# fdarmon/wild_deep_mvs

Hardware: AMD Instinct MI355X
Metric: cost-volume voxels/sec (BxDxHxW), MVSNet hot path (higher is better)
Workload: dtype bf16

## Files before the change

### wild_deep_mvs_amd/csrc/pscv_common.h

```cpp
#pragma once
#include <hip/hip_runtime.h>
#include <stdint.h>
#include <stdio.h>
#include <stdarg.h>

#include "../../include/pscv.h"

namespace pscv {

void set_error(const char* fmt, ...);

hipError_t ensure_dyn_lds(const void* kernel, int bytes);
int device_cu_count();

struct Knob {
    int process;
    int id;
    operator int() const;
    void set(int v) { __atomic_store_n(&process, v, __ATOMIC_RELAXED); }
};
#define PSCV_KNOB_TABLE(X)                      \
    X("warp_q2", g_warp_q2, 1)                  \
    X("warp_lpv", g_warp_lpv_override, 0)       \
    X("warp_ppd", g_warp_ppd_override, 0)       \
    X("warp_tiled", g_warp_tiled, 1)            \
    X("warp_tile", g_warp_tile, 0)              \
    X("warp_gc_lds", g_warp_gc_lds, 1)          \
    X("warp_lds_pad", g_warp_lds_pad, 0)        \
    X("warp_bwd_direct", g_warp_bwd_direct, 0)  \
    X("sweep_dc", g_sweep_dc, 0)                \
    X("sweepc_slots", g_sweepc_slots, 0)        \
    X("sweepc_pd", g_sweepc_pd, 0)              \
    X("sweep_th16", g_sweep_th16, 0)            \
    X("sweep_kdm", g_sweep_kdm, 0)              \
    X("sweep_kdm_pd", g_sweep_kdm_pd, 0)        \
    X("c1_sweep", g_c1_sweep, 1)                \
    X("c1_nb", g_c1_nb, 0)                      \
    X("conv_s2_sweep", g_conv_s2_sweep, 1)      \
    X("s2s_slots", g_s2s_slots, 0)              \
    X("block8_slots", g_block8_slots, 0)        \
    X("conv2d_wlds", g_conv2d_wlds, 1)          \
// ... 264 lines not shown
```

### wild_deep_mvs_amd/csrc/pscv_host.cpp

```cpp
#include <stdarg.h>
#include <stdio.h>
#include <string.h>

#include <functional>
#include <mutex>
#include <unordered_map>

#include "pscv_common.h"

namespace pscv {

namespace {
struct DynLdsKey {
    const void* kernel;
    int dev;
    bool operator==(const DynLdsKey& o) const { return kernel == o.kernel && dev == o.dev; }
};
struct DynLdsHash {
    size_t operator()(const DynLdsKey& k) const { return std::hash<const void*>()(k.kernel) * 31u + std::hash<int>()(k.dev); }
};
struct DynLdsSlot { const void* kernel; int dev; int bytes; };
constexpr int DYN_LDS_SLOTS = 64;
thread_local DynLdsSlot g_dyn_lds_tl[DYN_LDS_SLOTS];
}
// ... 37 lines not shown
}

int device_cu_count() {
    constexpr int MAXDEV = 64;
    static int cached[MAXDEV];
    int dev = 0;
    if (hipGetDevice(&dev) != hipSuccess) return -1;
    if (dev >= 0 && dev < MAXDEV) {
        const int c = __atomic_load_n(&cached[dev], __ATOMIC_RELAXED);
        if (c > 0) return c;
    }
    int n = 0;
    if (hipDeviceGetAttribute(&n, hipDeviceAttributeMultiprocessorCount, dev) != hipSuccess || n <= 0) return -1;
    if (dev >= 0 && dev < MAXDEV) __atomic_store_n(&cached[dev], n, __ATOMIC_RELAXED);
    return n;
}

static thread_local char g_err[512] = "";

void set_error(const char* fmt, ...) {
    va_list ap;
    va_start(ap, fmt);
    vsnprintf(g_err, sizeof(g_err), fmt, ap);
    va_end(ap);
}

#define PSCV_KNOB_ID(key, sym, def) KNOB_##sym,
enum { PSCV_KNOB_TABLE(PSCV_KNOB_ID) KNOB_COUNT };
#undef PSCV_KNOB_ID
#define PSCV_KNOB_DEFINE(key, sym, def) Knob sym = {def, KNOB_##sym};
// ... 211 lines not shown
```

### wild_deep_mvs_amd/csrc/warp_common.h

```cpp
#pragma once
#include "pscv_common.h"

namespace pscv {

struct WarpArgs {
    const void* ref;
    const void* src[PSCV_MAX_SRC];
    const float* cams;
    const float* depth;
    void* out;
    long depth_bstride;
    long out_view_stride;
    int n_src, B, h, w, hs, ws, D;
    int depth_per_pixel;
    int ppd;
    int npb_batch;
    int n_dchunks;
    int variant;
    float temp;
    float sx, sy;
    float xlo, xhi, ylo, yhi;
    int ref_y0;
    int* mode_hist;
};

template <int N> struct VecF { float v[N]; };

template <typename T, int CPL> __device__ __forceinline__ VecF<CPL> load_chan(const T* p) {
    VecF<CPL> r;
#pragma unroll
    for (int k = 0; k < CPL / 8; ++k) {
        const f32x8 t = Elem<T>::load8(p + 8 * k);
#pragma unroll
        for (int j = 0; j < 8; ++j) r.v[8 * k + j] = t.v[j];
    }
    return r;
}
// ... 154 lines not shown
```

### wild_deep_mvs_amd/csrc/warp_cost.hip

```cpp
#include <string.h>

#include "warp_common.h"

namespace pscv {

template <typename TIn, typename TOut, int C, int LPV, int GEOM, int COST>
__global__ __launch_bounds__(256, 4) void warp_cost_kernel(const WarpArgs a) {
    constexpr int CPL = C / LPV;
    constexpr int PPB = 256 / LPV;
    constexpr int PIXB = C * (int)sizeof(TIn);
    constexpr int RQ = (GEOM == PSCV_GEOM_HOMOG) ? 2 : 1;
    static_assert(CPL % 8 == 0, "a lane owns whole 8-channel groups");

    const int wg = xcd_remap(blockIdx.x, gridDim.x);
    const int pb = __builtin_amdgcn_readfirstlane(wg / a.n_dchunks);
    const int dc = __builtin_amdgcn_readfirstlane(wg - pb * a.n_dchunks);

    const int b = __builtin_amdgcn_readfirstlane(pb / a.npb_batch);
    const int pbb = __builtin_amdgcn_readfirstlane(pb - b * a.npb_batch);

    const int tid = threadIdx.x;
    __shared__ float cam_lds[PSCV_MAX_SRC * PSCV_CAM_FLOATS];
    extern __shared__ __attribute__((aligned(16))) float4 ray_lds[];
    for (int i = tid; i < a.n_src * PSCV_CAM_FLOATS; i += 256) {
// ... 248 lines not shown
extern "C" int pscv_warp_cost_rows(const void* ref, const void* const* srcs, int n_src, const float* cams,
                                   const float* depth, long depth_bstride, int depth_per_pixel, int geom, int cost,
                                   float temp, void* out, int B, int C, int h, int w, int hs, int ws, int D, int in_dtype,
                                   int out_dtype, int ref_y0, void* stream) {
    using namespace pscv;
    PSCV_CHECK_ARG(ref_y0 >= 0 && ref_y0 < (1 << 20), "pscv_warp_cost_rows: ref_y0=%d", ref_y0);
    PSCV_CHECK_ARG(n_src >= 1 && n_src <= PSCV_MAX_SRC, "pscv_warp_cost: n_src=%d outside [1,%d]", n_src, PSCV_MAX_SRC);
    PSCV_CHECK_ARG(srcs && cams && depth && out, "pscv_warp_cost: null pointer argument");
    PSCV_CHECK_ARG(cost == PSCV_COST_WARP_ONLY || cost == PSCV_COST_VARIANCE_PARTIAL || ref, "pscv_warp_cost: ref is required for cost mode %d", cost);
    PSCV_CHECK_ARG(cost != PSCV_COST_VARIANCE_PARTIAL || out_dtype == PSCV_F32, "pscv_warp_cost: partial sums are written in fp32");
    PSCV_CHECK_ARG(B > 0 && h > 0 && w > 0 && hs > 1 && ws > 1 && D > 0, "pscv_warp_cost: bad sizes");
    PSCV_CHECK_ARG(C % 8 == 0, "pscv_warp_cost: C=%d must be a multiple of 8", C);
    PSCV_CHECK_ARG((long)hs * ws < (1L << 24) && (long)hs * ws * C * 4 < (1L << 32), "pscv_warp_cost: source map %dx%dx%d too large", hs, ws, C);
    WarpArgs a;
    a.mode_hist = nullptr;
    a.ref_y0 = ref_y0;
    a.ref = ref;
    for (int i = 0; i < PSCV_MAX_SRC; ++i) a.src[i] = i < n_src ? srcs[i] : nullptr;
    for (int i = 0; i < n_src; ++i) PSCV_CHECK_ARG(srcs[i], "pscv_warp_cost: srcs[%d] is null", i);
    a.cams = cams;
    a.depth = depth;
    a.out = out;
    a.depth_bstride = depth_bstride;
    a.n_src = n_src; a.B = B; a.h = h; a.w = w; a.hs = hs; a.ws = ws; a.D = D;
    a.depth_per_pixel = depth_per_pixel;
    a.temp = temp;
    a.variant = 0;
    const long vol = (long)B * D * h * w;
    a.out_view_stride = cost == PSCV_COST_GROUPCORR ? vol * (C / 4) : vol * C;
    if (geom == PSCV_GEOM_PROJ) {
// ... 27 lines not shown
```

### wild_deep_mvs_amd/csrc/warp_cost_tiled.hip

```cpp
#include <type_traits>

#include "warp_common.h"
#include "warp_lds.h"

namespace pscv {

#ifndef WL_TILE_H
#define WL_TILE_H 4
#endif
constexpr int WL_T = 8;
constexpr int WL_TH = WL_TILE_H;
constexpr int WL_THREADS = 64 * WL_TH;
constexpr int WL_PG = WL_TH / 2;
constexpr int WL_ARENA = WL_TH == 8 ? 636 : 316;
constexpr int WL_HI = WL_ARENA * 64;
constexpr int WL_STAGE_ROWS = 8;
constexpr int WL_BOX_H = WL_STAGE_ROWS * (WL_THREADS / 64 / WL_MAX_SRC);
constexpr int WL_NSETS = 7;
constexpr int WL_TABLE = 2 * WL_HI;
constexpr int WL_LDS = WL_TABLE + WL_NSETS * WL_MAX_SRC * 16 + 32;
static_assert(WL_LDS <= (WL_TH == 8 ? 81920 : 40960), "two / four blocks per CU");


__device__ __forceinline__ void wl_blend8(const wl_f4 (&t)[8], const float (&w)[4], float (&o)[8]) {
    o[0] = t[0].x * w[0]; o[1] = t[0].y * w[0]; o[2] = t[0].z * w[0]; o[3] = t[0].w * w[0];
    o[4] = t[1].x * w[0]; o[5] = t[1].y * w[0]; o[6] = t[1].z * w[0]; o[7] = t[1].w * w[0];
#pragma unroll
    for (int k = 1; k < 4; ++k) {
        o[0] = fmaf(t[2 * k].x, w[k], o[0]); o[1] = fmaf(t[2 * k].y, w[k], o[1]);
        o[2] = fmaf(t[2 * k].z, w[k], o[2]); o[3] = fmaf(t[2 * k].w, w[k], o[3]);
        o[4] = fmaf(t[2 * k + 1].x, w[k], o[4]); o[5] = fmaf(t[2 * k + 1].y, w[k], o[5]);
        o[6] = fmaf(t[2 * k + 1].z, w[k], o[6]); o[7] = fmaf(t[2 * k + 1].w, w[k], o[7]);
    }
}

__device__ __forceinline__ wl_f4 wl_tap(const unsigned char* lsm, unsigned off) { return *reinterpret_cast<const wl_f4*>(lsm + off); }

template <typename TOut> __device__ __forceinline__ void wl_store8(char* p, const float (&o)[8]) {
    if constexpr (sizeof(TOut) == 4) {
        *reinterpret_cast<float4*>(p) = make_float4(o[0], o[1], o[2], o[3]);
        *reinterpret_cast<float4*>(p + 16) = make_float4(o[4], o[5], o[6], o[7]);
    } else {
        *reinterpret_cast<uint4*>(p) = make_uint4(wl_pack2<TOut>(o[0], o[1]), wl_pack2<TOut>(o[2], o[3]),
                                                   wl_pack2<TOut>(o[4], o[5]), wl_pack2<TOut>(o[6], o[7]));
    }
}


template <typename TIn, typename TOut, int GEOM, int COST>
__global__ __launch_bounds__(WL_THREADS, 4) void warp_cost_lds_kernel(const WarpArgs a) {
    constexpr int C = 32, PIXB = 64;
    constexpr int OB = (int)sizeof(TOut);
    constexpr bool VAR = COST == PSCV_COST_VARIANCE || COST == PSCV_COST_VARIANCE_CVP;
    static_assert(GEOM == PSCV_GEOM_PROJ, "PROJ geometry (three depth-independent ray terms per (view, pixel))");
    extern __shared__ __attribute__((aligned(16))) unsigned char lsm[];

    const int dc = blockIdx.y;
    int b, tyi, txi;
    if (!wl_tile_decode<WL_T, WL_TH>(a, b, tyi, txi)) return;

    __builtin_amdgcn_s_setprio(3);
    __builtin_amdgcn_s_setreg((1 - 1) << 11 | 23 << 6 | 1, 1);
    const int tid = threadIdx.x;
    const int wave = __builtin_amdgcn_readfirstlane(tid >> 6), lane = tid & 63;
    const int x0t = txi * WL_T, y0t = tyi * WL_TH;
    const int d0 = dc * a.ppd, d1 = min(a.D, d0 + a.ppd);
    const float* const depth_b = a.depth + (long)b * a.depth_bstride;
    const int n_src = a.n_src;
    int* const table = reinterpret_cast<int*>(lsm + WL_TABLE);

    const float dlane = depth_b[min(d0 + lane, d1 - 1)];

    const int quad = lane >> 2, l = lane & 3;
    const int pl = (2 * (wave % WL_PG) + (quad >> 3)) * 8 + ((0x73261540u >> (4 * (quad & 7))) & 7);
// ... 8 lines not shown
    {
        const float* cam = a.cams + ((long)min(l, n_src - 1) * a.B + b) * PSCV_CAM_FLOATS;
        rx = fmaf(cam[1], py, cam[0] * px) + cam[2];
        ry = fmaf(cam[4], py, cam[3] * px) + cam[5];
        rz = fmaf(cam[7], py, cam[6] * px) + cam[8];
        tx = cam[9]; ty_ = cam[10]; tz = cam[11];
    }
    float rf[8], rf2[8];
    {
        const f32x8 t = Elem<TIn>::load8(reinterpret_cast<const TIn*>(a.ref) + ((long)b * hw + pflat) * C + l * 8);
#pragma unroll
        for (int j = 0; j < 8; ++j) { rf[j] = t.v[j]; rf2[j] = t.v[j] * t.v[j]; }
    }

    const int nplanes = d1 - d0;
    auto split_size = [](int m) { return m >= 4 ? ((m / 2 + 1) & ~1) : m; };
    const int hsz = split_size(nplanes);
    const int q0 = split_size(hsz), q2 = split_size(nplanes - hsz);
    if (wave < WL_MAX_SRC) {
        const int k = wave;
        const float inf = __builtin_inff();
        const bool inq0 = lane < q0, inq1 = lane >= q0 && lane < hsz, inq2 = lane >= hsz && lane < hsz + q2, inq3 = lane >= hsz + q2;
        const float qmin0 = wl_wave_reduce<false>(inq0 ? dlane : inf), qmax0 = wl_wave_reduce<true>(inq0 ? dlane : -inf);
        const float qmin1 = wl_wave_reduce<false>(inq1 ? dlane : inf), qmax1 = wl_wave_reduce<true>(inq1 ? dlane : -inf);
        const float qmin2 = wl_wave_reduce<false>(inq2 ? dlane : inf), qmax2 = wl_wave_reduce<true>(inq2 ? dlane : -inf);
        const float qmin3 = wl_wave_reduce<false>(inq3 ? dlane : inf), qmax3 = wl_wave_reduce<true>(inq3 ? dlane : -inf);
        const float dmin1 = fminf(qmin0, qmin1), dmax1 = fmaxf(qmax0, qmax1);
        const float dmin2 = hsz < nplanes ? fminf(qmin2, qmin3) : dmin1, dmax2 = hsz < nplanes ? fmaxf(qmax2, qmax3) : dmax1;
        const float dmin0 = fminf(dmin1, dmin2), dmax0 = fmaxf(dmax1, dmax2);
        const int set = min(lane >> 3, WL_NSETS - 1);
        const int corner = lane & 7;
        const float cx = (corner & 1) ? (float)min(x0t + WL_T - 1, a.w - 1) : (float)x0t;
        const float cy = (float)(((corner & 2) ? min(y0t + WL_TH - 1, a.h - 1) : y0t) + a.ref_y0);
        const float dlo = set == 0 ? dmin0 : set == 1 ? dmin1 : set == 2 ? dmin2 : set == 3 ? qmin0 : set == 4 ? qmin1 : set == 5 ? qmin2 : qmin3;
        const float dhi = set == 0 ? dmax0 : set == 1 ? dmax1 : set == 2 ? dmax2 : set == 3 ? qmax0 : set == 4 ? qmax1 : set == 5 ? qmax2 : qmax3;
        const float d = (corner & 4) ? dhi : dlo;
        int cX0 = 0, cY0 = 0, cX1 = -1, cY1 = -1, pitch = 4, mode = WL_ZERO;
        if (k < n_src) {
            typedef const __attribute__((address_space(4))) float* wl_cf;
            wl_cf cam = (wl_cf)(a.cams + ((long)k * a.B + b) * PSCV_CAM_FLOATS);
            const float ax = fmaf(cam[1], cy, cam[0] * cx) + cam[2];
            const float ay = fmaf(cam[4], cy, cam[3] * cx) + cam[5];
            const float az = fmaf(cam[7], cy, cam[6] * cx) + cam[8];
            const float hx = fmaf(ax, d, cam[9]), hy = fmaf(ay, d, cam[10]), hz = fmaf(az, d, cam[11]);
            const float inv_z = __builtin_amdgcn_rcpf(hz);
            const float u = hx * inv_z, v = hy * inv_z;
            const float okf = (hz > 1e-6f && fabsf(u) < 1e6f && fabsf(v) < 1e6f) ? 1.0f : 0.0f;
            const float umin = wl_reduce8<false>(u), umax = wl_reduce8<true>(u);
            const float vmin = wl_reduce8<false>(v), vmax = wl_reduce8<true>(v);
            const bool ok = wl_reduce8<false>(okf) != 0.0f;
            const float sl = 1.0f / 32.0f;
            const int X0 = (int)floorf(umin - sl), X1 = (int)floorf(umax + sl) + 1;
            const int Y0 = (int)floorf(vmin - sl), Y1 = (int)floorf(vmax + sl) + 1;
            mode = WL_DIRECT;
            if (ok) {
                const bool outside = X1 < 0 || Y1 < 0 || X0 > a.ws - 1 || Y0 > a.hs - 1;
                const bool inside = X0 >= 0 && Y0 >= 0 && X1 <= a.ws - 1 && Y1 <= a.hs - 1;
                cX0 = max(X0, 0); cX1 = min(X1, a.ws - 1); cY0 = max(Y0, 0); cY1 = min(Y1, a.hs - 1);
                const int bw = cX1 - cX0 + 1, bh = cY1 - cY0 + 1;
                pitch = (bw + 3) & ~3;
                if (outside) { mode = WL_ZERO; cX0 = 0; cY0 = 0; cX1 = -1; cY1 = -1; pitch = 4; }
                else if (bw <= 16 && bh <= WL_BOX_H) mode = inside ? WL_FAST : WL_GEN;
                else { cX0 = 0; cY0 = 0; cX1 = -1; cY1 = -1; pitch = 4; }
            } else { cX0 = 0; cY0 = 0; cX1 = -1; cY1 = -1; pitch = 4; }
        }
        if (corner == 0 && lane < 8 * WL_NSETS)
            *reinterpret_cast<uint4*>(table + (set * WL_MAX_SRC + k) * 4) =
                make_uint4(((unsigned)cX0 & 0xffffu) | ((unsigned)cY0 << 16), ((unsigned)cX1 & 0xffffu) | ((unsigned)cY1 << 16),
                           (unsigned)pitch | ((unsigned)mode << 16), 0u);
    }
    __syncthreads();

    int bPitch[WL_MAX_SRC], bMode[WL_MAX_SRC], bBase[WL_MAX_SRC], bX0[WL_MAX_SRC], bY0[WL_MAX_SRC], bX1[WL_MAX_SRC], bY1[WL_MAX_SRC];
    bool any_gen = false;
    auto read_records = [&](int set) -> bool {
        int used = 0;
        bool direct = false;
        any_gen = false;
#pragma unroll
        for (int k = 0; k < WL_MAX_SRC; ++k) {
            const uint4 rec = *reinterpret_cast<const uint4*>(table + (set * WL_MAX_SRC + k) * 4);
            const int rx = __builtin_amdgcn_readfirstlane((int)rec.x), ry = __builtin_amdgcn_readfirstlane((int)rec.y);
            const int rz = __builtin_amdgcn_readfirstlane((int)rec.z);
            bX0[k] = (short)(rx & 0xffff); bY0[k] = rx >> 16;
            bX1[k] = (short)(ry & 0xffff); bY1[k] = ry >> 16;
            bPitch[k] = rz & 0xffff;
            int mode = rz >> 16;
            const int need = bPitch[k] * (bY1[k] - bY0[k] + 1);
            if ((mode == WL_FAST || mode == WL_GEN) && used + need > WL_ARENA) mode = WL_DIRECT;
            bBase[k] = used;
            if (mode == WL_FAST || mode == WL_GEN) used += need;
            bMode[k] = mode;
            any_gen = any_gen || mode == WL_GEN;
            direct = direct || (k < n_src && mode == WL_DIRECT);
        }
        return direct;
    };
    unsigned long plan = 0;
    int nseg = 0;
    auto push = [&](int set, int pa, int pb) { plan |= (unsigned long)((unsigned)set | (unsigned)pa << 3 | (unsigned)pb << 9) << (16 * nseg); ++nseg; };
    if (!read_records(0) || !(hsz < nplanes) || a.variant == 1) {
        push(0, 0, nplanes);
    } else {
        const bool quarters = a.variant != 3;
        if (read_records(1) && q0 < hsz && quarters) { push(3, 0, q0); push(4, q0, hsz); } else push(1, 0, hsz);
        if (read_records(2) && q2 < nplanes - hsz && quarters) { push(5, hsz, hsz + q2); push(6, hsz + q2, nplanes); } else push(2, hsz, nplanes);
    }
    for (int sub = 0; sub < nseg; ++sub) {
    const unsigned seg = (unsigned)(plan >> (16 * sub)) & 0xffffu;
    if (sub) {
        __syncthreads();
        __builtin_amdgcn_s_setprio(3);
    }
    read_records((int)(seg & 7u));
    const int s0 = d0 + (int)((seg >> 3) & 63u), s1 = d0 + (int)(seg >> 9);
    if (a.mode_hist && tid == 0) {
#pragma unroll
        for (int k = 0; k < WL_MAX_SRC; ++k)
            if (k < n_src) atomicAdd(a.mode_hist + k * 4 + bMode[k], 1);
    }
    const int sel = l;
    int mX0 = bX0[0], mY0 = bY0[0], mX1 = bX1[0], mY1 = bY1[0], mpitch = bPitch[0], mbase = bBase[0];
#pragma unroll
    for (int k = 1; k < WL_MAX_SRC; ++k)
        if (sel == k) { mX0 = bX0[k]; mY0 = bY0[k]; mX1 = bX1[k]; mY1 = bY1[k]; mpitch = bPitch[k]; mbase = bBase[k]; }
    const int meb = mbase - mY0 * mpitch - mX0;

    {
        constexpr int WPV = WL_THREADS / 64 / WL_MAX_SRC;
// ... 190 lines not shown
            for (int j = 0; j < 8; ++j) { const float m = __fmul_rn(invN, s[j]); o[j] = fmaf(invN, q[j], -__fmul_rn(m, m)); }
        } else {
            const float inv = 1.0f / (sum_e + 1e-6f);
#pragma unroll
            for (int j = 0; j < 8; ++j) o[j] = s[j] * inv;
        }
#pragma unroll
        for (int j = 0; j < 8; ++j) asm volatile("" : "+v"(o[j]));
        if (active) wl_store8<TOut>(out + ((unsigned long)b * a.D + d) * plane_bytes + lane_out, o);
    }
    }
}

template <typename TIn, typename TOut, int COST>
static int wl_launch(const WarpArgs& a, dim3 grid, hipStream_t st) {
    const int lds = min(WL_LDS + 1024 * max(0, (int)g_warp_lds_pad), 160 * 1024);
    return launch("pscv_warp_cost(lds)", warp_cost_lds_kernel<TIn, TOut, PSCV_GEOM_PROJ, COST>, grid, dim3(WL_THREADS), lds, st, a);
}

template <typename TIn, typename TOut>
static int wl_dispatch(const WarpArgs& a, int cost, dim3 grid, hipStream_t st) {
    if (cost == PSCV_COST_VARIANCE) return wl_launch<TIn, TOut, PSCV_COST_VARIANCE>(a, grid, st);
    if (cost == PSCV_COST_VARIANCE_CVP) return wl_launch<TIn, TOut, PSCV_COST_VARIANCE_CVP>(a, grid, st);
    if (cost == PSCV_COST_SOFTMIN) return wl_launch<TIn, TOut, PSCV_COST_SOFTMIN>(a, grid, st);
    return 1;
}

int* g_wl_mode_hist = nullptr;

int warp_cost_tiled_try(WarpArgs& a, int C, int geom, int cost, int in_dtype, int out_dtype, int ppd_override, hipStream_t st) {
    if (a.depth_per_pixel || geom != PSCV_GEOM_PROJ) return 1;
    if (out_dtype != in_dtype && out_dtype != PSCV_F32) return 1;
    if (a.n_src < 1 || a.n_src > WL_MAX_SRC) return 1;
    dim3 grid;
    const int rc = wl_plan("pscv_warp_cost(lds)", a, C, in_dtype, WL_T, WL_TH, ppd_override, a.D >= 96 ? 48 : 32, 64, grid);
    if (rc) return rc;
    a.variant = g_warp_tile;
    a.mode_hist = g_wl_mode_hist;
    return with_warp_types<false>("pscv_warp_cost(lds)", in_dtype, out_dtype, [&](auto ti, auto to) {
        return wl_dispatch<typename decltype(ti)::type, typename decltype(to)::type>(a, cost, grid, st);
    });
}

}

extern "C" void pscv_debug_wl_mode_hist(int* hist) { pscv::g_wl_mode_hist = hist; }
extern "C" int pscv_debug_wl_occupancy(int* blocks_per_cu, int* lds_bytes, int* threads) {
    auto kern = pscv::warp_cost_lds_kernel<pscv::f16_t, pscv::f16_t, PSCV_GEOM_PROJ, PSCV_COST_VARIANCE>;
    (void)pscv::ensure_dyn_lds(reinterpret_cast<const void*>(kern), pscv::WL_LDS);
    *lds_bytes = pscv::WL_LDS;
    *threads = pscv::WL_THREADS;
    return (int)hipOccupancyMaxActiveBlocksPerMultiprocessor(blocks_per_cu, kern, pscv::WL_THREADS, pscv::WL_LDS);
}
```

### wild_deep_mvs_amd/csrc/warp_lds.h

```cpp
#pragma once
#include "warp_common.h"

namespace pscv {

constexpr int WL_MAX_SRC = 4;
typedef float wl_f4 __attribute__((ext_vector_type(4)));

template <int CTRL> __device__ __forceinline__ int wl_dpp_i(int x) { return __builtin_amdgcn_mov_dpp(x, CTRL, 0xf, 0xf, true); }
template <int CTRL> __device__ __forceinline__ float wl_dpp_f(float x) {
    return __builtin_bit_cast(float, wl_dpp_i<CTRL>(__builtin_bit_cast(int, x)));
}


template <bool MAX> __device__ __forceinline__ float wl_mm(float a, float b) { return MAX ? fmaxf(a, b) : fminf(a, b); }
template <bool MAX, int CTRL, int ROWMASK = 0xf> __device__ __forceinline__ float wl_red_step(float x) {
    const int xi = __builtin_bit_cast(int, x);
    const float y = __builtin_bit_cast(float, __builtin_amdgcn_update_dpp(xi, xi, CTRL, ROWMASK, 0xf, false));
    return wl_mm<MAX>(x, y);
}
template <bool MAX> __device__ __forceinline__ float wl_reduce8(float x) {
    x = wl_red_step<MAX, 0xB1>(x);
    x = wl_red_step<MAX, 0x4E>(x);
    return wl_red_step<MAX, 0x141>(x);
}
// ... 9 lines not shown
    if constexpr (Half16<TOut>::dtype == PSCV_F16) {
        h2_t v;
        v[0] = (_Float16)lo;
        v[1] = (_Float16)hi;
        return __builtin_bit_cast(uint32_t, v);
    } else {
        return Half16<TOut>::pack(lo, hi);
    }
}
constexpr int WL_DIRECT = 0;
constexpr int WL_GEN = 1;
constexpr int WL_FAST = 2;
constexpr int WL_ZERO = 3;


template <int T, int TH> __device__ __forceinline__ bool wl_tile_decode(const WarpArgs& a, int& b, int& tyi, int& txi) {
    const int tpx = gridDim.x >> 3;
    const int ntx = (a.w + T - 1) / T, nty = (a.h + TH - 1) / TH;
    const int tile = ((int)blockIdx.x & 7) * tpx + ((int)blockIdx.x >> 3);
    if (tile >= a.B * nty * ntx) return false;
    const int trow = (int)(((float)tile + 0.5f) * (1.0f / (float)ntx));
    txi = tile - trow * ntx;
    b = (int)(((float)trow + 0.5f) * (1.0f / (float)nty));
    tyi = trow - b * nty;
    return true;
}

inline int wl_plan(const char* what, WarpArgs& a, int C, int in_dtype, int T, int TH, int ppd_override, int ppd_default, int ppd_max, dim3& grid) {
    if (C != 32 || (in_dtype != PSCV_F16 && in_dtype != PSCV_BF16)) return 1;
    if (a.ws > 16384 || a.hs > 16384) return 1;
    const long tiles = (long)a.B * ((a.h + TH - 1) / TH) * ((a.w + T - 1) / T);
    if (tiles >= (1L << 22)) return 1;
    int ppd = ppd_override > 0 ? min((ppd_override + 1) & ~1, ppd_max) : ppd_default;
    while (ppd > 4 && tiles * ((a.D + ppd - 1) / ppd) < 1024) ppd >>= 1;
    a.ppd = ppd;
    a.n_dchunks = (a.D + ppd - 1) / ppd;
    const long nblk = tiles * a.n_dchunks;
    if (nblk <= 0 || nblk > 0x7fffffffL) { set_error("%s: bad grid %ld", what, nblk); return -1; }
    grid = dim3(8 * (unsigned)((tiles + 7) / 8), a.n_dchunks);
    return 0;
// ... 4 lines not shown
```

### wild_deep_mvs_amd/graph.py

```python
from __future__ import annotations

from typing import Any, Dict, Tuple

import torch
import torch.nn as nn


def _sig(x) -> Any:
    if isinstance(x, torch.Tensor):
        return ("T", tuple(x.shape), str(x.dtype), str(x.device))
    if isinstance(x, (list, tuple)):
        return (type(x).__name__,) + tuple(_sig(v) for v in x)
    if isinstance(x, dict):
        return ("D",) + tuple((k, _sig(v)) for k, v in sorted(x.items()))
    return ("V", repr(x))


def _clone_static(x):
    if isinstance(x, torch.Tensor):
        return x.detach().clone()
    if isinstance(x, (list, tuple)):
        return type(x)(_clone_static(v) for v in x)
    if isinstance(x, dict):
        return {k: _clone_static(v) for k, v in x.items()}
# ... 49 lines not shown
        wkey = _weights_key(self.model)
        entry = self._graphs.get(key)
        if entry is not None and entry[3] != wkey:
            entry = None
        if entry is None:
            static_args, static_kwargs = _clone_static(args), _clone_static(kwargs)
            with torch.no_grad():
                side = torch.cuda.Stream()
                side.wait_stream(torch.cuda.current_stream())
                with torch.cuda.stream(side):
                    for _ in range(self.warmup):
                        self.model(*static_args, **static_kwargs)
                torch.cuda.current_stream().wait_stream(side)
                torch.cuda.synchronize()
                graph = torch.cuda.CUDAGraph()
                with torch.cuda.graph(graph, capture_error_mode="thread_local"):
                    static_out = self.model(*static_args, **static_kwargs)
            entry = (graph, (static_args, static_kwargs), static_out, wkey)
            self._graphs[key] = entry
        graph, (static_args, static_kwargs), static_out, _ = entry
        _copy_in(static_args, args)
        _copy_in(static_kwargs, kwargs)
        graph.replay()
        return _clone_out(static_out)


import functools
import operator
import sys
import threading
from collections import OrderedDict
# ... 112 lines not shown
                    state["seen"][key] = True
                    while len(state["seen"]) > 64:
                        state["seen"].popitem(last=False)
                    eager = True
            if not eager and entry is None:
                static_args, static_kwargs = _clone_static(args), _clone_static(kwargs)
                try:
                    with torch.no_grad():
                        side = torch.cuda.Stream()
                        side.wait_stream(torch.cuda.current_stream())
                        with torch.cuda.stream(side):
                            forward(self, *static_args, **static_kwargs)
                        torch.cuda.current_stream().wait_stream(side)
                        torch.cuda.synchronize()
                        graph = torch.cuda.CUDAGraph()
                        with torch.cuda.graph(graph, capture_error_mode="thread_local"):
                            static_out = forward(self, *static_args, **static_kwargs)
                except Exception:
                    state["failed"].add(key)
                    torch.cuda.synchronize()
                    eager = True
                else:
                    entry = (graph, (static_args, static_kwargs), static_out, wkey)
                    state["graphs"][key] = entry
                    while len(state["graphs"]) > MAX_GRAPHS_PER_MODEL:
                        old_key, _ = state["graphs"].popitem(last=False)
                        n = state["evicted"][old_key] = state["evicted"].get(old_key, 0) + 1
                        if n >= MAX_EVICTIONS_PER_SIGNATURE:
                            state["failed"].add(old_key)
            elif not eager:
                state["graphs"].move_to_end(key)
# ... 60 lines not shown
```

Measured before the change: 13.19 billion.

## Precompute per-tile source bounding boxes in a separate kernel table

Adds a pre-pass kernel that computes, for each tile and depth chunk, the projected source-view boxes, LDS arena allocation and sweep plan, and writes them to a global workspace table. The tiled warp-cost kernel gets a TABLE variant that reads these records from scalar memory. This removes the per-block wave reductions, projection math and the __syncthreads before the sweep, and it shrinks the LDS footprint. The cost is an extra launch, a cached per-stream workspace allocation, and a fallback when the stream is capturing. Graph capture is also moved to the side stream, so the workspace lookup is keyed on that stream.

```diff
diff --git a/wild_deep_mvs_amd/csrc/pscv_common.h b/wild_deep_mvs_amd/csrc/pscv_common.h
--- a/wild_deep_mvs_amd/csrc/pscv_common.h
+++ b/wild_deep_mvs_amd/csrc/pscv_common.h
@@ -12,6 +12,7 @@
 
 hipError_t ensure_dyn_lds(const void* kernel, int bytes);
 int device_cu_count();
+void* stream_workspace(hipStream_t st, size_t bytes);
 
 struct Knob {
     int process;
@@ -25,6 +26,7 @@
     X("warp_ppd", g_warp_ppd_override, 0)       \
     X("warp_tiled", g_warp_tiled, 1)            \
     X("warp_tile", g_warp_tile, 0)              \
+    X("warp_boxes", g_warp_boxes, 1)            \
     X("warp_gc_lds", g_warp_gc_lds, 1)          \
     X("warp_lds_pad", g_warp_lds_pad, 0)        \
     X("warp_bwd_direct", g_warp_bwd_direct, 0)  \
diff --git a/wild_deep_mvs_amd/csrc/pscv_host.cpp b/wild_deep_mvs_amd/csrc/pscv_host.cpp
--- a/wild_deep_mvs_amd/csrc/pscv_host.cpp
+++ b/wild_deep_mvs_amd/csrc/pscv_host.cpp
@@ -75,6 +75,25 @@
     if (hipDeviceGetAttribute(&n, hipDeviceAttributeMultiprocessorCount, dev) != hipSuccess || n <= 0) return -1;
     if (dev >= 0 && dev < MAXDEV) __atomic_store_n(&cached[dev], n, __ATOMIC_RELAXED);
     return n;
+}
+
+void* stream_workspace(hipStream_t st, size_t bytes) {
+    struct Buf { void* p; size_t bytes; };
+    static std::mutex mu;
+    static std::unordered_map<DynLdsKey, Buf, DynLdsHash> bufs;
+    int dev = 0;
+    if (hipGetDevice(&dev) != hipSuccess) return nullptr;
+    std::lock_guard<std::mutex> lk(mu);
+    Buf& buf = bufs[DynLdsKey{st, dev}];
+    if (buf.bytes >= bytes) return buf.p;
+    hipStreamCaptureStatus cs = hipStreamCaptureStatusNone;
+    if (hipStreamIsCapturing(st, &cs) != hipSuccess) { (void)hipGetLastError(); return nullptr; }
+    if (cs != hipStreamCaptureStatusNone) return nullptr;
+    const size_t want = (bytes + bytes / 2 + 0xffff) & ~(size_t)0xffff;
+    void* p = nullptr;
+    if (hipMalloc(&p, want) != hipSuccess) { (void)hipGetLastError(); return nullptr; }
+    buf = Buf{p, want};
+    return p;
 }
 
 static thread_local char g_err[512] = "";
diff --git a/wild_deep_mvs_amd/csrc/warp_boxes.hip b/wild_deep_mvs_amd/csrc/warp_boxes.hip
--- /dev/null
+++ b/wild_deep_mvs_amd/csrc/warp_boxes.hip
@@ -0,0 +1,76 @@
+#include "warp_common.h"
+#include "warp_lds.h"
+
+namespace pscv {
+
+struct WlBoxArgs {
+    const float* cams;
+    const float* depth;
+    int* table;
+    long depth_bstride;
+    int n_src, B, h, w, hs, ws, D, ppd, ref_y0, variant;
+    int T, TH, ntx, nty, arena, box_h;
+};
+
+constexpr int WB_WAVES = 4;
+constexpr int WB_TILES = 1;
+
+__global__ __launch_bounds__(64 * WB_WAVES) void warp_box_table_kernel(const WlBoxArgs a) {
+    const int dc = blockIdx.y, b = blockIdx.z;
+    const int lane = threadIdx.x & 63, wave = __builtin_amdgcn_readfirstlane((int)threadIdx.x >> 6);
+    const int d0 = dc * a.ppd, d1 = min(a.D, d0 + a.ppd);
+    const int nplanes = d1 - d0;
+    const float dlane = (a.depth + (long)b * a.depth_bstride)[min(d0 + lane, d1 - 1)];
+    WlCam cm[WL_MAX_SRC];
+#pragma unroll
+    for (int k = 0; k < WL_MAX_SRC; ++k) cm[k] = wl_load_cam(a.cams, k, a.n_src, a.B, b);
+    const int hsz = wl_split_size(nplanes);
+    const int q0 = wl_split_size(hsz), q2 = wl_split_size(nplanes - hsz);
+    float dlo, dhi;
+    wl_depth_ranges(dlane, lane, nplanes, hsz, q0, q2, dlo, dhi);
+    const int set = min(lane >> 3, WL_NSETS - 1), corner = lane & 7;
+    const int tpi = a.ntx * a.nty;
+    const long ntiles = (long)a.B * tpi;
+    for (int t = blockIdx.x * WB_WAVES + wave; t < tpi; t += gridDim.x * WB_WAVES) {
+        const int tyi = t / a.ntx, txi = t - tyi * a.ntx;
+        const int x0t = txi * a.T, y0t = tyi * a.TH;
+        uint4 rec[WL_MAX_SRC];
+        int used = 0;
+        bool direct = false, any_gen = false;
+#pragma unroll
+        for (int k = 0; k < WL_MAX_SRC; ++k) {
+            const uint3 r = wl_corner_box(cm[k], k < a.n_src, corner, x0t, y0t,
+                                          a.T, a.TH, dlo, dhi, a.h, a.w, a.hs, a.ws, a.ref_y0, a.box_h);
+            const int rx = (int)r.x, ry = (int)r.y, rz = (int)r.z;
+            const int Y0 = rx >> 16, Y1 = ry >> 16, pitch = rz & 0xffff;
+            int mode = rz >> 16, base;
+            wl_alloc_view(k, a.n_src, a.arena, pitch, Y0, Y1, mode, base, used, any_gen, direct);
+            rec[k] = make_uint4(r.x, r.y, (unsigned)pitch | ((unsigned)mode << 16), (unsigned)base);
+        }
+        unsigned long plan;
+        int nseg;
+        wl_sweep_plan([&](int s) { return __builtin_amdgcn_readlane((int)direct, 8 * s) != 0; }, nplanes, hsz, q0, q2, a.variant, plan, nseg);
+        int* const out = a.table + ((long)dc * ntiles + (long)b * tpi + t) * WL_REC_INTS;
+        for (int j = 0; j < nseg; ++j) {
+            const int sset = (int)(plan >> (16 * j)) & 7;
+            if (lane == 8 * sset) {
+#pragma unroll
+                for (int k = 0; k < WL_MAX_SRC; ++k) *reinterpret_cast<uint4*>(out + (j * WL_MAX_SRC + k) * 4) = rec[k];
+            }
+        }
+        if (lane == 0) *reinterpret_cast<uint4*>(out + WL_REC_HDR) = make_uint4((unsigned)plan, (unsigned)(plan >> 32), (unsigned)nseg, 0u);
+    }
+}
+
+int warp_box_table(const WarpArgs& a, int T, int TH, int arena, int box_h, int* table, hipStream_t st) {
+    WlBoxArgs g;
+    g.cams = a.cams; g.depth = a.depth; g.table = table; g.depth_bstride = a.depth_bstride;
+    g.n_src = a.n_src; g.B = a.B; g.h = a.h; g.w = a.w; g.hs = a.hs; g.ws = a.ws; g.D = a.D; g.ppd = a.ppd; g.ref_y0 = a.ref_y0; g.variant = a.variant;
+    g.T = T; g.TH = TH; g.ntx = (a.w + T - 1) / T; g.nty = (a.h + TH - 1) / TH; g.arena = arena; g.box_h = box_h;
+    const int tpi = g.ntx * g.nty;
+    if (a.B > 65535 || a.n_dchunks > 65535) { set_error("pscv_warp_cost(boxes): grid %d x %d", a.n_dchunks, a.B); return -1; }
+    const dim3 grid((unsigned)((tpi + WB_WAVES * WB_TILES - 1) / (WB_WAVES * WB_TILES)), (unsigned)a.n_dchunks, (unsigned)a.B);
+    return launch("pscv_warp_cost(boxes)", warp_box_table_kernel, grid, dim3(64 * WB_WAVES), 0, st, g);
+}
+
+}
diff --git a/wild_deep_mvs_amd/csrc/warp_common.h b/wild_deep_mvs_amd/csrc/warp_common.h
--- a/wild_deep_mvs_amd/csrc/warp_common.h
+++ b/wild_deep_mvs_amd/csrc/warp_common.h
@@ -21,6 +21,7 @@
     float sx, sy;
     float xlo, xhi, ylo, yhi;
     int ref_y0;
+    const int* box_table;
     int* mode_hist;
 };
 
diff --git a/wild_deep_mvs_amd/csrc/warp_cost.hip b/wild_deep_mvs_amd/csrc/warp_cost.hip
--- a/wild_deep_mvs_amd/csrc/warp_cost.hip
+++ b/wild_deep_mvs_amd/csrc/warp_cost.hip
@@ -286,6 +286,7 @@
     PSCV_CHECK_ARG((long)hs * ws < (1L << 24) && (long)hs * ws * C * 4 < (1L << 32), "pscv_warp_cost: source map %dx%dx%d too large", hs, ws, C);
     WarpArgs a;
     a.mode_hist = nullptr;
+    a.box_table = nullptr;
     a.ref_y0 = ref_y0;
     a.ref = ref;
     for (int i = 0; i < PSCV_MAX_SRC; ++i) a.src[i] = i < n_src ? srcs[i] : nullptr;
diff --git a/wild_deep_mvs_amd/csrc/warp_cost_tiled.hip b/wild_deep_mvs_amd/csrc/warp_cost_tiled.hip
--- a/wild_deep_mvs_amd/csrc/warp_cost_tiled.hip
+++ b/wild_deep_mvs_amd/csrc/warp_cost_tiled.hip
@@ -16,10 +16,10 @@
 constexpr int WL_HI = WL_ARENA * 64;
 constexpr int WL_STAGE_ROWS = 8;
 constexpr int WL_BOX_H = WL_STAGE_ROWS * (WL_THREADS / 64 / WL_MAX_SRC);
-constexpr int WL_NSETS = 7;
+constexpr int WL_LDS = 2 * WL_HI + 32;
 constexpr int WL_TABLE = 2 * WL_HI;
-constexpr int WL_LDS = WL_TABLE + WL_NSETS * WL_MAX_SRC * 16 + 32;
-static_assert(WL_LDS <= (WL_TH == 8 ? 81920 : 40960), "two / four blocks per CU");
+constexpr int WL_LDS_SELF = WL_TABLE + WL_NSETS * WL_MAX_SRC * 16 + 32;
+static_assert(WL_LDS <= WL_LDS_SELF && WL_LDS_SELF <= (WL_TH == 8 ? 81920 : 40960), "two / four blocks per CU");
 
 
 __device__ __forceinline__ void wl_blend8(const wl_f4 (&t)[8], const float (&w)[4], float (&o)[8]) {
@@ -47,7 +47,7 @@
 }
 
 
-template <typename TIn, typename TOut, int GEOM, int COST>
+template <typename TIn, typename TOut, int GEOM, int COST, bool TABLE>
 __global__ __launch_bounds__(WL_THREADS, 4) void warp_cost_lds_kernel(const WarpArgs a) {
     constexpr int C = 32, PIXB = 64;
     constexpr int OB = (int)sizeof(TOut);
@@ -56,8 +56,8 @@
     extern __shared__ __attribute__((aligned(16))) unsigned char lsm[];
 
     const int dc = blockIdx.y;
-    int b, tyi, txi;
-    if (!wl_tile_decode<WL_T, WL_TH>(a, b, tyi, txi)) return;
+    int b, tyi, txi, tile, ntiles;
+    if (!wl_tile_decode<WL_T, WL_TH>(a, b, tyi, txi, tile, ntiles)) return;
 
     __builtin_amdgcn_s_setprio(3);
     __builtin_amdgcn_s_setreg((1 - 1) << 11 | 23 << 6 | 1, 1);
@@ -96,62 +96,23 @@
     }
 
     const int nplanes = d1 - d0;
-    auto split_size = [](int m) { return m >= 4 ? ((m / 2 + 1) & ~1) : m; };
-    const int hsz = split_size(nplanes);
-    const int q0 = split_size(hsz), q2 = split_size(nplanes - hsz);
+    const int hsz = wl_split_size(nplanes);
+    const int q0 = wl_split_size(hsz), q2 = wl_split_size(nplanes - hsz);
+    if constexpr (!TABLE) {
     if (wave < WL_MAX_SRC) {
         const int k = wave;
-        const float inf = __builtin_inff();
-        const bool inq0 = lane < q0, inq1 = lane >= q0 && lane < hsz, inq2 = lane >= hsz && lane < hsz + q2, inq3 = lane >= hsz + q2;
-        const float qmin0 = wl_wave_reduce<false>(inq0 ? dlane : inf), qmax0 = wl_wave_reduce<true>(inq0 ? dlane : -inf);
-        const float qmin1 = wl_wave_reduce<false>(inq1 ? dlane : inf), qmax1 = wl_wave_reduce<true>(inq1 ? dlane : -inf);
-        const float qmin2 = wl_wave_reduce<false>(inq2 ? dlane : inf), qmax2 = wl_wave_reduce<true>(inq2 ? dlane : -inf);
-        const float qmin3 = wl_wave_reduce<false>(inq3 ? dlane : inf), qmax3 = wl_wave_reduce<true>(inq3 ? dlane : -inf);
-        const float dmin1 = fminf(qmin0, qmin1), dmax1 = fmaxf(qmax0, qmax1);
-        const float dmin2 = hsz < nplanes ? fminf(qmin2, qmin3) : dmin1, dmax2 = hsz < nplanes ? fmaxf(qmax2, qmax3) : dmax1;
-        const float dmin0 = fminf(dmin1, dmin2), dmax0 = fmaxf(dmax1, dmax2);
+        float dlo, dhi;
+        wl_depth_ranges(dlane, lane, nplanes, hsz, q0, q2, dlo, dhi);
         const int set = min(lane >> 3, WL_NSETS - 1);
         const int corner = lane & 7;
-        const float cx = (corner & 1) ? (float)min(x0t + WL_T - 1, a.w - 1) : (float)x0t;
-        const float cy = (float)(((corner & 2) ? min(y0t + WL_TH - 1, a.h - 1) : y0t) + a.ref_y0);
-        const float dlo = set == 0 ? dmin0 : set == 1 ? dmin1 : set == 2 ? dmin2 : set == 3 ? qmin0 : set == 4 ? qmin1 : set == 5 ? qmin2 : qmin3;
-        const float dhi = set == 0 ? dmax0 : set == 1 ? dmax1 : set == 2 ? dmax2 : set == 3 ? qmax0 : set == 4 ? qmax1 : set == 5 ? qmax2 : qmax3;
-        const float d = (corner & 4) ? dhi : dlo;
-        int cX0 = 0, cY0 = 0, cX1 = -1, cY1 = -1, pitch = 4, mode = WL_ZERO;
-        if (k < n_src) {
-            typedef const __attribute__((address_space(4))) float* wl_cf;
-            wl_cf cam = (wl_cf)(a.cams + ((long)k * a.B + b) * PSCV_CAM_FLOATS);
-            const float ax = fmaf(cam[1], cy, cam[0] * cx) + cam[2];
-            const float ay = fmaf(cam[4], cy, cam[3] * cx) + cam[5];
-            const float az = fmaf(cam[7], cy, cam[6] * cx) + cam[8];
-            const float hx = fmaf(ax, d, cam[9]), hy = fmaf(ay, d, cam[10]), hz = fmaf(az, d, cam[11]);
-            const float inv_z = __builtin_amdgcn_rcpf(hz);
-            const float u = hx * inv_z, v = hy * inv_z;
-            const float okf = (hz > 1e-6f && fabsf(u) < 1e6f && fabsf(v) < 1e6f) ? 1.0f : 0.0f;
-            const float umin = wl_reduce8<false>(u), umax = wl_reduce8<true>(u);
-            const float vmin = wl_reduce8<false>(v), vmax = wl_reduce8<true>(v);
-            const bool ok = wl_reduce8<false>(okf) != 0.0f;
-            const float sl = 1.0f / 32.0f;
-            const int X0 = (int)floorf(umin - sl), X1 = (int)floorf(umax + sl) + 1;
-            const int Y0 = (int)floorf(vmin - sl), Y1 = (int)floorf(vmax + sl) + 1;
-            mode = WL_DIRECT;
-            if (ok) {
-                const bool outside = X1 < 0 || Y1 < 0 || X0 > a.ws - 1 || Y0 > a.hs - 1;
-                const bool inside = X0 >= 0 && Y0 >= 0 && X1 <= a.ws - 1 && Y1 <= a.hs - 1;
-                cX0 = max(X0, 0); cX1 = min(X1, a.ws - 1); cY0 = max(Y0, 0); cY1 = min(Y1, a.hs - 1);
-                const int bw = cX1 - cX0 + 1, bh = cY1 - cY0 + 1;
-                pitch = (bw + 3) & ~3;
-                if (outside) { mode = WL_ZERO; cX0 = 0; cY0 = 0; cX1 = -1; cY1 = -1; pitch = 4; }
-                else if (bw <= 16 && bh <= WL_BOX_H) mode = inside ? WL_FAST : WL_GEN;
-                else { cX0 = 0; cY0 = 0; cX1 = -1; cY1 = -1; pitch = 4; }
-            } else { cX0 = 0; cY0 = 0; cX1 = -1; cY1 = -1; pitch = 4; }
-        }
+        const uint3 rec = wl_corner_box(wl_load_cam(a.cams, k, n_src, a.B, b), k < n_src, corner, x0t, y0t, WL_T, WL_TH,
+                                        dlo, dhi, a.h, a.w, a.hs, a.ws, a.ref_y0, WL_BOX_H);
         if (corner == 0 && lane < 8 * WL_NSETS)
-            *reinterpret_cast<uint4*>(table + (set * WL_MAX_SRC + k) * 4) =
-                make_uint4(((unsigned)cX0 & 0xffffu) | ((unsigned)cY0 << 16), ((unsigned)cX1 & 0xffffu) | ((unsigned)cY1 << 16),
-                           (unsigned)pitch | ((unsigned)mode << 16), 0u);
+            *reinterpret_cast<uint4*>(table + (set * WL_MAX_SRC + k) * 4) = make_uint4(rec.x, rec.y, rec.z, 0u);
     }
     __syncthreads();
+    }
+    const wl_ci recp = (wl_ci)(a.box_table + ((long)dc * ntiles + tile) * (TABLE ? WL_REC_INTS : 0));
 
     int bPitch[WL_MAX_SRC], bMode[WL_MAX_SRC], bBase[WL_MAX_SRC], bX0[WL_MAX_SRC], bY0[WL_MAX_SRC], bX1[WL_MAX_SRC], bY1[WL_MAX_SRC];
     bool any_gen = false;
@@ -161,32 +122,32 @@
         any_gen = false;
 #pragma unroll
         for (int k = 0; k < WL_MAX_SRC; ++k) {
-            const uint4 rec = *reinterpret_cast<const uint4*>(table + (set * WL_MAX_SRC + k) * 4);
-            const int rx = __builtin_amdgcn_readfirstlane((int)rec.x), ry = __builtin_amdgcn_readfirstlane((int)rec.y);
-            const int rz = __builtin_amdgcn_readfirstlane((int)rec.z);
+            int rx, ry, rz;
+            if constexpr (TABLE) {
+                const wl_ci r = recp + (set * WL_MAX_SRC + k) * 4;
+                rx = r[0]; ry = r[1]; rz = r[2];
+                bBase[k] = r[3];
+            } else {
+                const uint4 rec = *reinterpret_cast<const uint4*>(table + (set * WL_MAX_SRC + k) * 4);
+                rx = __builtin_amdgcn_readfirstlane((int)rec.x); ry = __builtin_amdgcn_readfirstlane((int)rec.y);
+                rz = __builtin_amdgcn_readfirstlane((int)rec.z);
+            }
             bX0[k] = (short)(rx & 0xffff); bY0[k] = rx >> 16;
             bX1[k] = (short)(ry & 0xffff); bY1[k] = ry >> 16;
             bPitch[k] = rz & 0xffff;
-            int mode = rz >> 16;
-            const int need = bPitch[k] * (bY1[k] - bY0[k] + 1);
-            if ((mode == WL_FAST || mode == WL_GEN) && used + need > WL_ARENA) mode = WL_DIRECT;
-            bBase[k] = used;
-            if (mode == WL_FAST || mode == WL_GEN) used += need;
-            bMode[k] = mode;
-            any_gen = any_gen || mode == WL_GEN;
-            direct = direct || (k < n_src && mode == WL_DIRECT);
+            bMode[k] = rz >> 16;
+            if constexpr (TABLE) any_gen = any_gen || bMode[k] == WL_GEN;
+            else wl_alloc_view(k, n_src, WL_ARENA, bPitch[k], bY0[k], bY1[k], bMode[k], bBase[k], used, any_gen, direct);
         }
         return direct;
     };
-    unsigned long plan = 0;
-    int nseg = 0;
-    auto push = [&](int set, int pa, int pb) { plan |= (unsigned long)((unsigned)set | (unsigned)pa << 3 | (unsigned)pb << 9) << (16 * nseg); ++nseg; };
-    if (!read_records(0) || !(hsz < nplanes) || a.variant == 1) {
-        push(0, 0, nplanes);
+    unsigned long plan;
+    int nseg;
+    if constexpr (TABLE) {
+        plan = (unsigned long)(unsigned)recp[WL_REC_HDR] | (unsigned long)(unsigned)recp[WL_REC_HDR + 1] << 32;
+        nseg = recp[WL_REC_HDR + 2];
     } else {
-        const bool quarters = a.variant != 3;
-        if (read_records(1) && q0 < hsz && quarters) { push(3, 0, q0); push(4, q0, hsz); } else push(1, 0, hsz);
-        if (read_records(2) && q2 < nplanes - hsz && quarters) { push(5, hsz, hsz + q2); push(6, hsz + q2, nplanes); } else push(2, hsz, nplanes);
+        wl_sweep_plan(read_records, nplanes, hsz, q0, q2, a.variant, plan, nseg);
     }
     for (int sub = 0; sub < nseg; ++sub) {
     const unsigned seg = (unsigned)(plan >> (16 * sub)) & 0xffffu;
@@ -194,7 +155,7 @@
         __syncthreads();
         __builtin_amdgcn_s_setprio(3);
     }
-    read_records((int)(seg & 7u));
+    read_records(TABLE ? sub : (int)(seg & 7u));
     const int s0 = d0 + (int)((seg >> 3) & 63u), s1 = d0 + (int)(seg >> 9);
     if (a.mode_hist && tid == 0) {
 #pragma unroll
@@ -415,8 +376,10 @@
 
 template <typename TIn, typename TOut, int COST>
 static int wl_launch(const WarpArgs& a, dim3 grid, hipStream_t st) {
-    const int lds = min(WL_LDS + 1024 * max(0, (int)g_warp_lds_pad), 160 * 1024);
-    return launch("pscv_warp_cost(lds)", warp_cost_lds_kernel<TIn, TOut, PSCV_GEOM_PROJ, COST>, grid, dim3(WL_THREADS), lds, st, a);
+    const int pad = 1024 * max(0, (int)g_warp_lds_pad);
+    if (a.box_table)
+        return launch("pscv_warp_cost(lds)", warp_cost_lds_kernel<TIn, TOut, PSCV_GEOM_PROJ, COST, true>, grid, dim3(WL_THREADS), min(WL_LDS + pad, 160 * 1024), st, a);
+    return launch("pscv_warp_cost(lds)", warp_cost_lds_kernel<TIn, TOut, PSCV_GEOM_PROJ, COST, false>, grid, dim3(WL_THREADS), min(WL_LDS_SELF + pad, 160 * 1024), st, a);
 }
 
 template <typename TIn, typename TOut>
@@ -427,6 +390,7 @@
     return 1;
 }
 
+int warp_box_table(const WarpArgs& a, int T, int TH, int arena, int box_h, int* table, hipStream_t st);
 int* g_wl_mode_hist = nullptr;
 
 int warp_cost_tiled_try(WarpArgs& a, int C, int geom, int cost, int in_dtype, int out_dtype, int ppd_override, hipStream_t st) {
@@ -438,6 +402,16 @@
     if (rc) return rc;
     a.variant = g_warp_tile;
     a.mode_hist = g_wl_mode_hist;
+    a.box_table = nullptr;
+    if (g_warp_boxes) {
+        const long nrec = (long)(grid.x / 8) * 8 * a.n_dchunks;
+        int* const tab = static_cast<int*>(stream_workspace(st, (size_t)nrec * WL_REC_INTS * sizeof(int)));
+        if (tab) {
+            const int rb = warp_box_table(a, WL_T, WL_TH, WL_ARENA, WL_BOX_H, tab, st);
+            if (rb) return rb;
+            a.box_table = tab;
+        }
+    }
     return with_warp_types<false>("pscv_warp_cost(lds)", in_dtype, out_dtype, [&](auto ti, auto to) {
         return wl_dispatch<typename decltype(ti)::type, typename decltype(to)::type>(a, cost, grid, st);
     });
@@ -447,7 +421,7 @@
 
 extern "C" void pscv_debug_wl_mode_hist(int* hist) { pscv::g_wl_mode_hist = hist; }
 extern "C" int pscv_debug_wl_occupancy(int* blocks_per_cu, int* lds_bytes, int* threads) {
-    auto kern = pscv::warp_cost_lds_kernel<pscv::f16_t, pscv::f16_t, PSCV_GEOM_PROJ, PSCV_COST_VARIANCE>;
+    auto kern = pscv::warp_cost_lds_kernel<pscv::f16_t, pscv::f16_t, PSCV_GEOM_PROJ, PSCV_COST_VARIANCE, true>;
     (void)pscv::ensure_dyn_lds(reinterpret_cast<const void*>(kern), pscv::WL_LDS);
     *lds_bytes = pscv::WL_LDS;
     *threads = pscv::WL_THREADS;
diff --git a/wild_deep_mvs_amd/csrc/warp_lds.h b/wild_deep_mvs_amd/csrc/warp_lds.h
--- a/wild_deep_mvs_amd/csrc/warp_lds.h
+++ b/wild_deep_mvs_amd/csrc/warp_lds.h
@@ -47,16 +47,114 @@
 constexpr int WL_ZERO = 3;
 
 
-template <int T, int TH> __device__ __forceinline__ bool wl_tile_decode(const WarpArgs& a, int& b, int& tyi, int& txi) {
+constexpr int WL_NSETS = 7;
+constexpr int WL_MAX_SEG = 4;
+constexpr int WL_REC_HDR = WL_MAX_SEG * WL_MAX_SRC * 4;
+constexpr int WL_REC_INTS = WL_REC_HDR + 4;
+typedef const __attribute__((address_space(4))) float* wl_cf;
+typedef const __attribute__((address_space(4))) int* wl_ci;
+
+__device__ __forceinline__ int wl_split_size(int m) { return m >= 4 ? ((m / 2 + 1) & ~1) : m; }
+
+__device__ __forceinline__ void wl_depth_ranges(float dlane, int lane, int nplanes, int hsz, int q0, int q2, float& dlo, float& dhi) {
+    const float inf = __builtin_inff();
+    const bool inq0 = lane < q0, inq1 = lane >= q0 && lane < hsz, inq2 = lane >= hsz && lane < hsz + q2, inq3 = lane >= hsz + q2;
+    const float qmin0 = wl_wave_reduce<false>(inq0 ? dlane : inf), qmax0 = wl_wave_reduce<true>(inq0 ? dlane : -inf);
+    const float qmin1 = wl_wave_reduce<false>(inq1 ? dlane : inf), qmax1 = wl_wave_reduce<true>(inq1 ? dlane : -inf);
+    const float qmin2 = wl_wave_reduce<false>(inq2 ? dlane : inf), qmax2 = wl_wave_reduce<true>(inq2 ? dlane : -inf);
+    const float qmin3 = wl_wave_reduce<false>(inq3 ? dlane : inf), qmax3 = wl_wave_reduce<true>(inq3 ? dlane : -inf);
+    const float dmin1 = fminf(qmin0, qmin1), dmax1 = fmaxf(qmax0, qmax1);
+    const float dmin2 = hsz < nplanes ? fminf(qmin2, qmin3) : dmin1, dmax2 = hsz < nplanes ? fmaxf(qmax2, qmax3) : dmax1;
+    const float dmin0 = fminf(dmin1, dmin2), dmax0 = fmaxf(dmax1, dmax2);
+    const int set = min(lane >> 3, WL_NSETS - 1);
+    dlo = set == 0 ? dmin0 : set == 1 ? dmin1 : set == 2 ? dmin2 : set == 3 ? qmin0 : set == 4 ? qmin1 : set == 5 ? qmin2 : qmin3;
+    dhi = set == 0 ? dmax0 : set == 1 ? dmax1 : set == 2 ? dmax2 : set == 3 ? qmax0 : set == 4 ? qmax1 : set == 5 ? qmax2 : qmax3;
+}
+
+struct WlCam { float c[12]; };
+__device__ __forceinline__ WlCam wl_load_cam(const float* cams, int k, int n_src, int B, int b) {
+    const wl_cf p = (wl_cf)(cams + ((long)min(k, n_src - 1) * B + b) * PSCV_CAM_FLOATS);
+    WlCam r;
+#pragma unroll
+    for (int i = 0; i < 12; ++i) r.c[i] = p[i];
+    return r;
+}
+__device__ __forceinline__ uint3 wl_corner_box(const WlCam& cm, bool have, int corner, int x0t, int y0t, int T, int TH, float dlo, float dhi,
+                                               int h, int w, int hs, int ws, int ref_y0, int box_h) {
+    const float cx = (corner & 1) ? (float)min(x0t + T - 1, w - 1) : (float)x0t;
+    const float cy = (float)(((corner & 2) ? min(y0t + TH - 1, h - 1) : y0t) + ref_y0);
+    const float d = (corner & 4) ? dhi : dlo;
+    int cX0 = 0, cY0 = 0, cX1 = -1, cY1 = -1, pitch = 4, mode = WL_ZERO;
+    if (have) {
+        const float* const cam = cm.c;
+        const float ax = fmaf(cam[1], cy, cam[0] * cx) + cam[2];
+        const float ay = fmaf(cam[4], cy, cam[3] * cx) + cam[5];
+        const float az = fmaf(cam[7], cy, cam[6] * cx) + cam[8];
+        const float hx = fmaf(ax, d, cam[9]), hy = fmaf(ay, d, cam[10]), hz = fmaf(az, d, cam[11]);
+        const float inv_z = __builtin_amdgcn_rcpf(hz);
+        const float u = hx * inv_z, v = hy * inv_z;
+        const float okf = (hz > 1e-6f && fabsf(u) < 1e6f && fabsf(v) < 1e6f) ? 1.0f : 0.0f;
+        const float umin = wl_reduce8<false>(u), umax = wl_reduce8<true>(u);
+        const float vmin = wl_reduce8<false>(v), vmax = wl_reduce8<true>(v);
+        const bool ok = wl_reduce8<false>(okf) != 0.0f;
+        const float sl = 1.0f / 32.0f;
+        const int X0 = (int)floorf(umin - sl), X1 = (int)floorf(umax + sl) + 1;
+        const int Y0 = (int)floorf(vmin - sl), Y1 = (int)floorf(vmax + sl) + 1;
+        mode = WL_DIRECT;
+        if (ok) {
+            const bool outside = X1 < 0 || Y1 < 0 || X0 > ws - 1 || Y0 > hs - 1;
+            const bool inside = X0 >= 0 && Y0 >= 0 && X1 <= ws - 1 && Y1 <= hs - 1;
+            cX0 = max(X0, 0); cX1 = min(X1, ws - 1); cY0 = max(Y0, 0); cY1 = min(Y1, hs - 1);
+            const int bw = cX1 - cX0 + 1, bh = cY1 - cY0 + 1;
+            pitch = (bw + 3) & ~3;
+            if (outside) { mode = WL_ZERO; cX0 = 0; cY0 = 0; cX1 = -1; cY1 = -1; pitch = 4; }
+            else if (bw <= 16 && bh <= box_h) mode = inside ? WL_FAST : WL_GEN;
+            else { cX0 = 0; cY0 = 0; cX1 = -1; cY1 = -1; pitch = 4; }
+        } else { cX0 = 0; cY0 = 0; cX1 = -1; cY1 = -1; pitch = 4; }
+    }
+    return make_uint3(((unsigned)cX0 & 0xffffu) | ((unsigned)cY0 << 16), ((unsigned)cX1 & 0xffffu) | ((unsigned)cY1 << 16),
+                      (unsigned)pitch | ((unsigned)mode << 16));
+}
+
+__device__ __forceinline__ void wl_alloc_view(int k, int n_src, int arena, int pitch, int Y0, int Y1, int& mode, int& base, int& used,
+                                              bool& any_gen, bool& direct) {
+    const int need = pitch * (Y1 - Y0 + 1);
+    if ((mode == WL_FAST || mode == WL_GEN) && used + need > arena) mode = WL_DIRECT;
+    base = used;
+    if (mode == WL_FAST || mode == WL_GEN) used += need;
+    any_gen = any_gen || mode == WL_GEN;
+    direct = direct || (k < n_src && mode == WL_DIRECT);
+}
+
+template <typename F>
+__device__ __forceinline__ void wl_sweep_plan(F&& direct_of, int nplanes, int hsz, int q0, int q2, int variant, unsigned long& plan, int& nseg) {
+    plan = 0;
+    nseg = 0;
+    auto push = [&](int set, int pa, int pb) { plan |= (unsigned long)((unsigned)set | (unsigned)pa << 3 | (unsigned)pb << 9) << (16 * nseg); ++nseg; };
+    if (!direct_of(0) || !(hsz < nplanes) || variant == 1) {
+        push(0, 0, nplanes);
+    } else {
+        const bool quarters = variant != 3;
+        if (direct_of(1) && q0 < hsz && quarters) { push(3, 0, q0); push(4, q0, hsz); } else push(1, 0, hsz);
+        if (direct_of(2) && q2 < nplanes - hsz && quarters) { push(5, hsz, hsz + q2); push(6, hsz + q2, nplanes); } else push(2, hsz, nplanes);
+    }
+}
+
+template <int T, int TH> __device__ __forceinline__ bool wl_tile_decode(const WarpArgs& a, int& b, int& tyi, int& txi, int& tile, int& ntiles) {
     const int tpx = gridDim.x >> 3;
     const int ntx = (a.w + T - 1) / T, nty = (a.h + TH - 1) / TH;
-    const int tile = ((int)blockIdx.x & 7) * tpx + ((int)blockIdx.x >> 3);
-    if (tile >= a.B * nty * ntx) return false;
+    tile = ((int)blockIdx.x & 7) * tpx + ((int)blockIdx.x >> 3);
+    ntiles = a.B * nty * ntx;
+    if (tile >= ntiles) return false;
     const int trow = (int)(((float)tile + 0.5f) * (1.0f / (float)ntx));
     txi = tile - trow * ntx;
     b = (int)(((float)trow + 0.5f) * (1.0f / (float)nty));
     tyi = trow - b * nty;
     return true;
+}
+template <int T, int TH> __device__ __forceinline__ bool wl_tile_decode(const WarpArgs& a, int& b, int& tyi, int& txi) {
+    int tile, ntiles;
+    return wl_tile_decode<T, TH>(a, b, tyi, txi, tile, ntiles);
 }
 
 inline int wl_plan(const char* what, WarpArgs& a, int C, int in_dtype, int T, int TH, int ppd_override, int ppd_default, int ppd_max, dim3& grid) {
diff --git a/wild_deep_mvs_amd/graph.py b/wild_deep_mvs_amd/graph.py
--- a/wild_deep_mvs_amd/graph.py
+++ b/wild_deep_mvs_amd/graph.py
@@ -87,7 +87,7 @@
                 torch.cuda.current_stream().wait_stream(side)
                 torch.cuda.synchronize()
                 graph = torch.cuda.CUDAGraph()
-                with torch.cuda.graph(graph, capture_error_mode="thread_local"):
+                with torch.cuda.graph(graph, stream=side, capture_error_mode="thread_local"):
                     static_out = self.model(*static_args, **static_kwargs)
             entry = (graph, (static_args, static_kwargs), static_out, wkey)
             self._graphs[key] = entry
@@ -230,7 +230,7 @@
                         torch.cuda.current_stream().wait_stream(side)
                         torch.cuda.synchronize()
                         graph = torch.cuda.CUDAGraph()
-                        with torch.cuda.graph(graph, capture_error_mode="thread_local"):
+                        with torch.cuda.graph(graph, stream=side, capture_error_mode="thread_local"):
                             static_out = forward(self, *static_args, **static_kwargs)
                 except Exception:
                     state["failed"].add(key)
```

New measurement: 13.31 billion, median of 6. About the same (+0.9%).
